# ross39/new_bloom_filter_repo

Measured on AMD Instinct MI355X. Metric: Mpixels/s Bloom insert+query, 1080p residuals, higher is better.
Workload: dtype u64

## Files before the change

new_bloom_filter_repo_amd/csrc/rbf_api.hip:

```cpp
#include "rbf_host.h"
#include "rbf_kernels_noise.h"
#include "rbf_kernels_pack.h"
#include "rbf_rice_host.h"

#include <cmath>

struct MaskArgs {
    const void *frames; FrameLayout l; uint32_t nframes;
    int32_t thr_floor; const int32_t *thr_floors;
    void *masks; uint64_t mask_stride; uint64_t *ones;
    uint32_t channels;
};

static int launch_finish_ones(rbf_ctx *ctx, uint64_t *ones_dev, uint32_t pairs, uint64_t *host_block, uint64_t token,
                              void *clear_a, size_t bytes_a, void *clear_b, size_t bytes_b)
{
    if (clear_a && (((uintptr_t)clear_a | bytes_a) & 15)) { HIP_TRY(hipMemsetAsync(clear_a, 0, bytes_a, ctx->stream)); clear_a = nullptr; bytes_a = 0; }
    if (clear_b && (((uintptr_t)clear_b | bytes_b) & 15)) { HIP_TRY(hipMemsetAsync(clear_b, 0, bytes_b, ctx->stream)); clear_b = nullptr; bytes_b = 0; }
    const uint64_t quads = bytes_a / 16 + bytes_b / 16;
    uint32_t blocks = (uint32_t)((quads + 256 * 4 - 1) / (256 * 4));
    if (blocks < 1) blocks = 1;
    if (blocks > 1024) blocks = 1024;
    hipLaunchKernelGGL(k_finish_ones, dim3(blocks), dim3(256), 0, ctx->stream, ctx->ones_acc.p, ones_dev, pairs, host_block, token,
                       (uint4 *)clear_a, (uint64_t)(bytes_a / 16), (uint4 *)clear_b, (uint64_t)(bytes_b / 16));
// ... 575 lines not shown
    LaunchTimer t(ctx, scatter ? RBF_K_SCATTER : RBF_K_GATHER);
    if (int r = count_and_scan_masks(ctx, mask_dev, 0, n, 1, count_dev)) return r;
    by_sample_width(sample_bytes, [&](auto s) {
        using S = decltype(s);
        auto kern = scatter ? k_values<S, true> : k_values<S, false>;
        hipLaunchKernelGGL(kern, grid, block, 0, ctx->stream, (uint8_t *)frame_dev, width, n, row_pitch_bytes, pixel_stride_bytes, channels,
                           (const uint64_t *)mask_dev, ctx->seg_off.p, nseg, (S *)values_dev);
    });
    HIP_TRY(hipGetLastError());
    return RBF_OK;
}

extern "C" {

int rbf_version(void) { return RBF_ABI_VERSION; }
const char *rbf_last_error(void) { return g_err; }

int rbf_device_count(int *count)
{
    if (!count) return fail(RBF_EINVAL, "count is null");
    int c = 0;
    hipError_t e = hipGetDeviceCount(&c);
    if (e != hipSuccess) { *count = 0; return fail(RBF_EIO, "hipGetDeviceCount: %s", hipGetErrorString(e)); }
    *count = c;
    return RBF_OK;
}

int rbf_ctx_create(int device, void *hip_stream, rbf_ctx **out)
{
    if (!out) return fail(RBF_EINVAL, "out is null");
    *out = nullptr;
    int count = 0;
    HIP_TRY(hipGetDeviceCount(&count));
    if (device < 0 || device >= count) return fail(RBF_EINVAL, "device %d out of range (have %d)", device, count);
    HIP_TRY(hipSetDevice(device));
    rbf_ctx *c = new (std::nothrow) rbf_ctx();
    if (!c) return fail(RBF_ENOMEM, "out of host memory");
    c->device = device;
    int cus = 0;
    if (hipDeviceGetAttribute(&cus, hipDeviceAttributeMultiprocessorCount, device) == hipSuccess && cus > 0) c->cus = (uint32_t)cus;
    if (hip_stream) { c->stream = (hipStream_t)hip_stream; c->owns_stream = false; }
    else {
        hipError_t e = hipStreamCreateWithFlags(&c->stream, hipStreamNonBlocking);
        if (e != hipSuccess) { delete c; return fail(RBF_EIO, "hipStreamCreate: %s", hipGetErrorString(e)); }
        c->owns_stream = true;
    }
    *out = c;
    return RBF_OK;
}

int rbf_ctx_destroy(rbf_ctx *ctx)
{
    if (!ctx) return RBF_OK;
    (void)hipSetDevice(ctx->device);
    (void)hipStreamSynchronize(ctx->stream);
    for (auto &t : ctx->pending) { (void)hipEventDestroy(t.a); (void)hipEventDestroy(t.b); }
    for (auto e : ctx->pool) (void)hipEventDestroy(e);
    hash_table_release(ctx);
    if (ctx->owns_stream) (void)hipStreamDestroy(ctx->stream);
    delete ctx;
    return RBF_OK;
}

int rbf_ctx_sync(rbf_ctx *ctx)
{
    if (int r = set_device(ctx)) return r;
    HIP_TRY(hipStreamSynchronize(ctx->stream));
    return RBF_OK;
}

int rbf_malloc(rbf_ctx *ctx, size_t bytes, void **out_dev)
{
    if (int r = set_device(ctx)) return r;
    if (!out_dev) return fail(RBF_EINVAL, "out_dev is null");
    *out_dev = nullptr;
    if (bytes == 0) bytes = 8;
    hipError_t e = hipMalloc(out_dev, bytes);
    if (e != hipSuccess) return fail(e == hipErrorOutOfMemory ? RBF_ENOMEM : RBF_EIO, "hipMalloc(%zu): %s", bytes, hipGetErrorString(e));
    return RBF_OK;
}

int rbf_free(rbf_ctx *ctx, void *ptr_dev)
{
    if (int r = set_device(ctx)) return r;
    if (!ptr_dev) return RBF_OK;
    HIP_TRY(hipStreamSynchronize(ctx->stream));
    HIP_TRY(hipFree(ptr_dev));
    return RBF_OK;
}

int rbf_memset(rbf_ctx *ctx, void *dst_dev, int value, size_t bytes)
{
    if (int r = set_device(ctx)) return r;
    if (bytes == 0) return RBF_OK;
    if (!dst_dev) return fail(RBF_EINVAL, "dst_dev is null");
    HIP_TRY(hipMemsetAsync(dst_dev, value, bytes, ctx->stream));
    return RBF_OK;
}

int rbf_memcpy_h2d(rbf_ctx *ctx, void *dst_dev, const void *src, size_t bytes)
{
    if (int r = set_device(ctx)) return r;
    if (bytes == 0) return RBF_OK;
    if (!dst_dev || !src) return fail(RBF_EINVAL, "null pointer");
    HIP_TRY(hipMemcpyAsync(dst_dev, src, bytes, hipMemcpyHostToDevice, ctx->stream));
    HIP_TRY(hipStreamSynchronize(ctx->stream));
    return RBF_OK;
}

int rbf_memcpy_d2h(rbf_ctx *ctx, void *dst, const void *src_dev, size_t bytes)
{
    if (int r = set_device(ctx)) return r;
    if (bytes == 0) return RBF_OK;
    if (!dst || !src_dev) return fail(RBF_EINVAL, "null pointer");
    HIP_TRY(hipMemcpyAsync(dst, src_dev, bytes, hipMemcpyDeviceToHost, ctx->stream));
    HIP_TRY(hipStreamSynchronize(ctx->stream));
    return RBF_OK;
}

int rbf_memcpy_d2d(rbf_ctx *ctx, void *dst_dev, const void *src_dev, size_t bytes)
{
    if (int r = set_device(ctx)) return r;
    if (bytes == 0) return RBF_OK;
    if (!dst_dev || !src_dev) return fail(RBF_EINVAL, "null pointer");
    HIP_TRY(hipMemcpyAsync(dst_dev, src_dev, bytes, hipMemcpyDeviceToDevice, ctx->stream));
    return RBF_OK;
}

int rbf_timing_enable(rbf_ctx *ctx, int on)
{
    if (int r = set_device(ctx)) return r;
    if (!on) { if (int r = drain_timing(ctx)) return r; }
    ctx->timing = on == 1 ? 0xFFFFFFFFu : (uint32_t)on;
    return RBF_OK;
}

int rbf_ctx_force_generic(rbf_ctx *ctx, int on)
{
    if (!ctx) return fail(RBF_EINVAL, "null context");
    ctx->knobs.set_flags(on);
    return RBF_OK;
}

int rbf_ctx_option(rbf_ctx *ctx, int option, int64_t value)
{
    if (!ctx) return fail(RBF_EINVAL, "null context");
    switch (option) {
    case RBF_OPT_SEPARATE_FINISH: ctx->knobs.no_fused_finish = value != 0; return RBF_OK;
    case RBF_OPT_INSERT_SLICES: ctx->knobs.insert_slices = value < 0 ? 0u : (uint32_t)value; return RBF_OK;
    default: return fail(RBF_EINVAL, "unknown option %d", option);
    }
}

int rbf_timing_reset(rbf_ctx *ctx)
{
    if (int r = set_device(ctx)) return r;
    if (int r = drain_timing(ctx)) return r;
    for (int k = 0; k < RBF_K_COUNT; ++k) { ctx->total_ms[k] = 0; ctx->launches[k] = 0; }
    return RBF_OK;
}

int rbf_timing_read(rbf_ctx *ctx, int kernel_id, double *total_ms, uint64_t *launches)
{
    if (int r = set_device(ctx)) return r;
    if (kernel_id < 0 || kernel_id >= RBF_K_COUNT) return fail(RBF_EINVAL, "kernel id %d", kernel_id);
    if (int r = drain_timing(ctx)) return r;
    if (total_ms) *total_ms = ctx->total_ms[kernel_id];
    if (launches) *launches = ctx->launches[kernel_id];
    return RBF_OK;
}

int rbf_optimal_params(uint64_t n, uint64_t ones, double *k_out, uint64_t *l_out)
{
    if (!k_out || !l_out) return fail(RBF_EINVAL, "null output");
    *k_out = 0.0; *l_out = 0;
    if (n == 0 || ones > n) return fail(RBF_EINVAL, "need 0 <= ones <= n, n > 0");
    const double p = (double)ones / (double)n;
    if (p <= 0.0001) return RBF_OK;
    if (p >= 0.32453) return RBF_OK;
    const double q = 1 - p;
    const double L = std::log(2.0);
    const double k = std::log2(q * std::pow(L, 2.0) / p);
    if (std::isnan(k) || k <= 0) return RBF_OK;
    const double gamma = 1 / L;
    const double lf = p * (double)n * k * gamma;
    const uint64_t l = (uint64_t)lf;
    *k_out = k > 0.1 ? k : 0.1;
    *l_out = l > 1 ? l : 1;
    return RBF_OK;
}

int rbf_activation_threshold(double k_star, uint32_t *floor_k, uint64_t *threshold)
{
    if (!floor_k || !threshold) return fail(RBF_EINVAL, "null output");
    if (!(k_star >= 0.0) || k_star > 64.0) return fail(RBF_ERANGE, "k* = %g outside [0, 64]", k_star);
    const double fl = std::floor(k_star);
    *floor_k = (uint32_t)fl;
    const double pa = k_star - fl;
    if (!(pa > 0.0)) { *threshold = 0; return RBF_OK; }
    int ex;
    const double fr = std::frexp(pa, &ex);
    const uint64_t A = (uint64_t)std::ldexp(fr, 53);
    const int s = ex - 53 - 2;
    const uint64_t N = (A == (1ull << 52)) ? 4 * A - 1 : 4 * A - 2;
    const int sh = -s;
    if (sh >= 128) { *threshold = 1; return RBF_OK; }
    const unsigned __int128 X = (unsigned __int128)N * (unsigned __int128)0xFFFFFFFFFFFFFFFFull;
    *threshold = (uint64_t)(X >> sh) + 1;
    return RBF_OK;
}

int rbf_plan_batch(uint64_t n, const uint64_t *ones, uint32_t nframes, int guard_l_ge_n,
                   rbf_filter_params *params, double *k_out)
{
    if (!ones || !params) return fail(RBF_EINVAL, "null pointer");
    for (uint32_t f = 0; f < nframes; ++f) {
        double k = 0.0; uint64_t l = 0;
        if (int r = rbf_optimal_params(n, ones[f], &k, &l)) return r;
        const bool skip = (l == 0) || (guard_l_ge_n && l >= n) || l > 0xFFFFFFFFull;
        params[f].m = 0; params[f].floor_k = 0; params[f].threshold = 0;
        if (!skip) {
            params[f].m = (uint32_t)l;
            if (int r = rbf_activation_threshold(k, &params[f].floor_k, &params[f].threshold)) return r;
        }
        if (k_out) k_out[f] = skip ? 0.0 : k;
    }
    return RBF_OK;
}

int rbf_residual_mask_batch(rbf_ctx *ctx, const void *frames_dev, uint64_t frame_stride_bytes,
                            uint32_t nframes, uint32_t width, uint32_t height,
                            uint64_t row_pitch_bytes, uint32_t pixel_stride_bytes,
                            uint32_t sample_bytes, int32_t thr_floor, const int32_t *thr_floors,
                            void *masks_dev, uint64_t mask_stride_bytes, uint64_t *ones_dev)
{
    return rbf_residual_mask_batch_ex(ctx, frames_dev, frame_stride_bytes, nframes, width, height, row_pitch_bytes, pixel_stride_bytes, sample_bytes,
                                      thr_floor, thr_floors, masks_dev, mask_stride_bytes, ones_dev, 1);
}

int rbf_residual_mask_batch_ex(rbf_ctx *ctx, const void *frames_dev, uint64_t frame_stride_bytes,
                               uint32_t nframes, uint32_t width, uint32_t height,
                               uint64_t row_pitch_bytes, uint32_t pixel_stride_bytes,
                               uint32_t sample_bytes, int32_t thr_floor, const int32_t *thr_floors,
                               void *masks_dev, uint64_t mask_stride_bytes, uint64_t *ones_dev, uint32_t mask_channels)
{
    const FrameLayout l{width, height, row_pitch_bytes, pixel_stride_bytes, sample_bytes, frame_stride_bytes};
    return residual_mask_impl(ctx, MaskArgs{frames_dev, l, nframes, thr_floor, thr_floors, masks_dev, mask_stride_bytes, ones_dev, mask_channels}, true);
}

int rbf_bgr_to_gray_batch(rbf_ctx *ctx, const void *frames_dev, uint64_t frame_stride_bytes, uint32_t nframes,
                          uint32_t width, uint32_t height, uint64_t row_pitch_bytes, uint32_t pixel_stride_bytes,
                          uint32_t sample_bytes, void *gray_dev)
{
    const FrameLayout l{width, height, row_pitch_bytes, pixel_stride_bytes, sample_bytes, frame_stride_bytes};
    return pixel_pass(ctx, frames_dev, l, nframes, 3, gray_dev, RBF_K_MASK, [](auto s) { return k_bgr_to_gray<decltype(s)>; });
}

int rbf_extract_luma_batch(rbf_ctx *ctx, const void *frames_dev, uint64_t frame_stride_bytes, uint32_t nframes,
                           uint32_t width, uint32_t height, uint64_t row_pitch_bytes, uint32_t pixel_stride_bytes,
                           uint32_t sample_bytes, void *luma_dev)
{
    const FrameLayout l{width, height, row_pitch_bytes, pixel_stride_bytes, sample_bytes, frame_stride_bytes};
    return pixel_pass(ctx, frames_dev, l, nframes, 1, luma_dev, -1, [](auto s) { return k_extract_luma<decltype(s)>; });
}

int rbf_noise_moments_batch(rbf_ctx *ctx, const void *frames_dev, uint64_t frame_stride_bytes,
                            uint32_t nframes, uint32_t width, uint32_t height,
                            uint64_t row_pitch_bytes, uint32_t pixel_stride_bytes,
                            uint32_t sample_bytes, int64_t *moments_dev, float *noise_dev)
{
    if (int r = set_device(ctx)) return r;
    if (!frames_dev || !moments_dev) return fail(RBF_EINVAL, "null device pointer");
    const FrameLayout l{width, height, row_pitch_bytes, pixel_stride_bytes, sample_bytes, frame_stride_bytes};
    if (int r = check_layout(l, nframes, frame_pass_rules(1))) return r;
    if ((uint64_t)width * height >= (1ull << 32)) return fail(RBF_ERANGE, "frame of %llu pixels is too large", (unsigned long long)width * height);
    const uint32_t by = (height + NZ_TILE_H - 1) / NZ_TILE_H;
    if (by > 65535) return fail(RBF_ERANGE, "frame height %u too large", height);
    HIP_TRY(hipMemsetAsync(moments_dev, 0, (size_t)nframes * 2 * sizeof(int64_t), ctx->stream));
    const dim3 grid((width + NZ_TILE_W - 1) / NZ_TILE_W, by, nframes), block(NZ_THREADS);
    LaunchTimer t(ctx, RBF_K_NOISE);
    by_sample_width(sample_bytes, [&](auto s) {
        hipLaunchKernelGGL(k_noise_moments<decltype(s)>, grid, block, 0, ctx->stream, (const uint8_t *)frames_dev, frame_stride_bytes, width, height,
                           row_pitch_bytes, pixel_stride_bytes, (unsigned long long *)moments_dev, noise_dev);
    });
    HIP_TRY(hipGetLastError());
    return RBF_OK;
}

int rbf_bloom_encode_batch(rbf_ctx *ctx, const void *masks_dev, uint64_t mask_stride_bytes,
                           uint64_t n, uint32_t nframes, const rbf_filter_params *params,
                           const rbf_seeds *seeds,
                           void *filters_dev, uint64_t filter_stride_bytes,
                           void *witnesses_dev, uint64_t witness_stride_bytes,
                           uint64_t *stats_dev)
{
    return encode_batch_impl(ctx, BloomBatch{(void *)masks_dev, mask_stride_bytes, n, nframes, params, seeds, filters_dev, filter_stride_bytes,
                                             witnesses_dev, witness_stride_bytes, stats_dev}, false);
}

int rbf_encode_gop(rbf_ctx *ctx, const void *frames_dev, uint64_t frame_stride_bytes,
                   uint32_t nframes, uint32_t width, uint32_t height,
                   uint64_t row_pitch_bytes, uint32_t pixel_stride_bytes,
                   uint32_t sample_bytes, int32_t thr_floor, const int32_t *thr_floors,
                   const rbf_seeds *seeds,
                   void *masks_dev, uint64_t mask_stride_bytes, uint64_t *ones_dev,
                   void *filters_dev, uint64_t filter_stride_bytes,
// ... 461 lines not shown
```

new_bloom_filter_repo_amd/csrc/rbf_kernels_i64.h:

```cpp
#pragma once
#include "rbf_kernels_q64.h"

namespace rbf {

constexpr int HT_THREADS = 256;

__global__ __launch_bounds__(HT_THREADS) void k_hash_table(uint64_t n, Seeds seeds, uint4 *__restrict__ table)
{
    const uint32_t lane = threadIdx.x & 63u, wave = threadIdx.x >> 6;
    const uint64_t seg = (uint64_t)blockIdx.x * (HT_THREADS / WAVE) + wave;
    if (seg * QL_SEG_PIXELS >= n) return;
    const uint64_t i0 = seg * QL_SEG_PIXELS + (uint64_t)lane * QL_P;
    uint64_t h1[QL_P], h2[QL_P], ha[QL_P];
    uint32_t validmask = 0;
#pragma unroll
    for (int it = 0; it < QL_P; ++it) {
        h1[it] = 0; h2[it] = 0; ha[it] = 0;
        if (i0 + it < n) validmask |= 1u << it;
    }
    if (!hash3_run8((uint32_t)i0, validmask, seeds, h1, h2, ha)) {
#pragma unroll
        for (int it = 0; it < QL_P; ++it) {
            const bool act = (validmask >> it) & 1u;
            const Hash3 h = hash3_index((uint32_t)(i0 + it), act, seeds);
            h1[it] = h.h1; h2[it] = h.h2; ha[it] = h.ha;
        }
    }
    hash_table_store8(table, n, seg, lane, h1, h2, ha);
}

constexpr int IT_STEP_BYTES = 128;
constexpr int IT_CHUNK_STEPS = 16;
constexpr int IT_QUEUE = 64 + IT_STEP_BYTES * 8;
constexpr int IT_STAGE_BYTES = IT_CHUNK_STEPS * IT_STEP_BYTES;
constexpr int IT_WAVE_LDS_BYTES = IT_QUEUE * 2 + IT_STAGE_BYTES;
static_assert(IT_WAVE_LDS_BYTES % 16 == 0 && (IT_QUEUE * 2) % 16 == 0, "the stage is written by LDS-DMA");

template <bool RECORDS, int NWAVES, bool HASHED = false, bool WHOLE = false>
__device__ __forceinline__ void insert_tab_steps(const uint8_t *__restrict__ mask , uint64_t row_bytes , uint64_t n,
                                                 const FrameDev &fd, const uint4 *__restrict__ table, const Seeds &seeds,
                                                 uint32_t *filt, uint32_t tile_bit0, uint32_t tile_bits, uint2 *__restrict__ records, uint32_t rpos,
                                                 uint32_t *wave_lds , uint64_t g0, uint64_t g1, uint32_t lane, uint32_t wave)
{
    static_assert((NWAVES & (NWAVES - 1)) == 0, "a power of two");
    uint16_t *q = reinterpret_cast<uint16_t *>(wave_lds);
    const uint32_t stage = __builtin_amdgcn_readfirstlane(lds_addr_of(wave_lds) + IT_QUEUE * 2);
    uint32_t qn = 0;
    const uint32_t m = vgpr_copy(__builtin_amdgcn_readfirstlane(fd.m));
    const uint32_t fk = __builtin_amdgcn_readfirstlane(fd.floor_k);
    const double ninv = __builtin_bit_cast(double, fd.M);
    const uint64_t T = fd.T;
    auto set_bit = [&](uint32_t pos) {
        if (WHOLE) { atomicOr(&filt[pos >> 5], msb_bit(pos)); return; }
        const uint32_t rel = pos - tile_bit0;
        if (rel < tile_bits) atomicOr(&filt[rel >> 5], msb_bit(pos));
    };

    const HashTable tv(const_cast<uint4 *>(table), n);
    const uint32_t Ttag = (uint32_t)(T >> 48);
    uint4 e0 = make_uint4(0, 0, 0, 0);
    uint32_t tag = 0, slot_kept = 0;
    uint64_t ha_kept = 0;
    uint32_t pending = 0;
    uint32_t cb = 0;
    auto fetch = [&](uint32_t first, uint32_t count) {
        const uint32_t e = lane < count ? q[first + lane] : 0u;
        const uint32_t idx = ((cb + (e >> 10) * NWAVES) << 10) + (e & 1023u);
        if (HASHED) {
            const Hash3 h = hash3_index(idx, lane < count, seeds);
            e0 = make_uint4((uint32_t)h.h1, (uint32_t)(h.h1 >> 32), (uint32_t)h.h2, (uint32_t)(h.h2 >> 32));
            tag = (uint32_t)(h.ha >> 48);
            ha_kept = h.ha;
        } else {
            slot_kept = hash_table_slot(idx);
            e0 = tv.pos[slot_kept];
            tag = tv.tag[idx];
        }
        pending = count;
    };
    auto finish = [&]() {
        if (!pending) return;
        if (lane < pending) {
            uint32_t pos = mod_m_f64(rn_double(e0.x, e0.y), e0.x, ninv, m);
            const uint32_t step = mod_m_f64(rn_double(e0.z, e0.w), e0.z, ninv, m);
            bool act = tag < Ttag;
            if (tag == Ttag) act = (HASHED ? ha_kept : tv.act[slot_kept]) < T;
            if (RECORDS) {
                records[rpos + lane] = make_uint2(pos, step | (act ? 0x80000000u : 0u));
            } else {
                for (uint32_t j = 0; j < fk; ++j) {
                    set_bit(pos);
                    const uint32_t s2 = pos + step;
                    pos = min(s2, s2 - m);
                }
                if (act) set_bit(pos);
            }
        }
        if (RECORDS) rpos += pending;
        pending = 0;
    };

    const uint32_t nbytes32 = (uint32_t)((n + 7) >> 3), n32 = (uint32_t)n, row32 = (uint32_t)row_bytes;
    const uint32_t gend = (uint32_t)g1;
    auto staged = [&](uint32_t s) -> uint32_t {
        return *reinterpret_cast<const __attribute__((address_space(3))) uint16_t *>((uintptr_t)(stage + s * IT_STEP_BYTES + lane * 2u));
    };
    auto decode = [&](uint32_t v, uint32_t g) -> uint32_t {
        const uint32_t byte = g * IT_STEP_BYTES + lane * 2u;
        const uint32_t x = __builtin_bitreverse32(v) >> 16;
        uint32_t b = ((x & 0xFFu) << 8) | (x >> 8);
        const uint32_t rem = n32 - byte * 8u;
        if (rem < 16u) b &= (1u << rem) - 1u;
        return (g < gend && byte < nbytes32) ? b : 0u;
    };
    for (uint32_t chunk = __builtin_amdgcn_readfirstlane((uint32_t)g0 + wave); chunk < gend; chunk += NWAVES * IT_CHUNK_STEPS) {
        cb = chunk;
        wave_lds_fence();
#pragma unroll
        for (int i = 0; i < IT_CHUNK_STEPS / 2; ++i) {
            const uint32_t g = cb + (2u * i + (lane >> 5)) * NWAVES;
            const uint32_t off = g * IT_STEP_BYTES + (lane & 31u) * 4u;
            if (g < gend && off < row32) {
                const uint32_t dst = stage + (uint32_t)i * 256u;
                uint32_t keep;
                asm volatile("s_mov_b32 %0, m0\n\ts_mov_b32 m0, %1\n\ts_nop 0\n\tglobal_load_lds_dword %2, %3\n\ts_mov_b32 m0, %0"
                             : "=&s"(keep) : "s"(dst), "v"(off), "s"(mask) : "memory");
            }
        }
        dma_wait_all();
        wave_lds_fence();
        uint32_t nxt = staged(0);
        for (uint32_t s = 0; s < IT_CHUNK_STEPS && cb + s * NWAVES < gend; ++s) {
            const uint32_t g = cb + s * NWAVES;
            uint32_t bits = decode(nxt, g);
            nxt = staged(s + 1 < IT_CHUNK_STEPS ? s + 1 : s);
            const uint32_t c = __popc(bits);
            const uint32_t incl = wave_inclusive_scan(c);
            const uint32_t excl = incl - c;
            const uint32_t total = __builtin_amdgcn_readlane(incl, 63);
            uint32_t off = qn + excl;
            const uint32_t ebase = (s << 10) | (lane << 4);
            while (bits) {
                q[off++] = (uint16_t)(ebase + __builtin_ctz(bits));
                bits &= bits - 1u;
            }
            qn += total;
            wave_lds_fence();
            while (qn >= WAVE) {
                qn -= WAVE;
                finish();
                fetch(qn, WAVE);
            }
            wave_lds_fence();
        }
        if (cb + NWAVES * IT_CHUNK_STEPS < gend && qn) {
            finish();
            fetch(0, qn);
            qn = 0;
            wave_lds_fence();
        }
    }
    finish();
    if (qn) { fetch(0, qn); finish(); }
}

template <bool HASHED = false, bool WHOLE = false>
__global__ __launch_bounds__(IL_THREADS) void k_insert_tab(
    const uint8_t *__restrict__ masks, uint64_t mask_stride_bytes, uint64_t n,
    const FrameTable tab, const uint4 *__restrict__ table , Seeds seeds,
    uint32_t *__restrict__ partials, uint64_t part_stride_words32, uint32_t tile_words ,
    const SliceTable slices, uint32_t per_tile , uint32_t Smax )
{
    extern __shared__ __attribute__((aligned(16))) uint32_t lds[];
    uint32_t *filt = lds;
    uint32_t *queues = lds + tile_words;
    const uint32_t tile = blockIdx.x / per_tile;
    uint32_t s = blockIdx.x - tile * per_tile, f = 0;
    while (s >= slices.n[f]) { s -= slices.n[f]; ++f; }
    const uint32_t S = slices.n[f];
    const FrameDev fd = tab.f[f];
    if (fd.m == 0) return;
    const uint32_t lane = threadIdx.x & 63u, wave = threadIdx.x >> 6;
    const uint32_t fwords = filter_words(fd.m);
    const uint32_t tile0 = tile * tile_words;
    if (tile0 >= fwords) return;
    for (uint32_t i = threadIdx.x; i < tile_words; i += IL_THREADS) filt[i] = 0;
    __syncthreads();

    const uint64_t nbytes = (n + 7) >> 3;
    const uint64_t groups = (nbytes + IT_STEP_BYTES - 1) / IT_STEP_BYTES;
    const uint64_t gper = (groups + S - 1) / S;
    const uint64_t g0 = (uint64_t)s * gper;
    const uint64_t g1 = g0 + gper < groups ? g0 + gper : groups;
    insert_tab_steps<false, IL_WAVES, HASHED, WHOLE>(masks + (uint64_t)f * mask_stride_bytes, mask_stride_bytes, n, fd, table, seeds, filt, tile0 << 5, tile_words << 5, nullptr, 0u,
                                                     queues + wave * (IT_WAVE_LDS_BYTES / 4), g0, g1, lane, wave);
    __syncthreads();
    uint32_t *part = partials + ((uint64_t)f * Smax + s) * part_stride_words32 + tile0;
    const uint32_t mine = fwords - tile0 < tile_words ? fwords - tile0 : tile_words;
    const uint32_t pairs = (mine + 1) >> 1;
    for (uint32_t i = threadIdx.x; i < pairs; i += IL_THREADS)
        reinterpret_cast<uint2 *>(part)[i] = reinterpret_cast<const uint2 *>(filt)[i];
}

constexpr int IP_THREADS = 256, IP_WAVES = IP_THREADS / WAVE;

template <bool HASHED = false>
__global__ __launch_bounds__(IP_THREADS) void k_insert_positions(
    const uint8_t *__restrict__ masks, uint64_t mask_stride_bytes, uint64_t n,
    const FrameTable tab , const uint4 *__restrict__ table , Seeds seeds,
    uint2 *__restrict__ records, uint32_t *__restrict__ counters )
{
    __shared__ __attribute__((aligned(16))) uint32_t queues[IP_WAVES * (IT_WAVE_LDS_BYTES / 4)];
    const uint32_t f = blockIdx.y, s = blockIdx.x, S = gridDim.x;
    const FrameDev fd = tab.f[f];
    if (fd.m == 0) return;
    const uint32_t lane = threadIdx.x & 63u, wave = threadIdx.x >> 6;
    const uint64_t nbytes = (n + 7) >> 3;
    const uint64_t groups = (nbytes + IT_STEP_BYTES - 1) / IT_STEP_BYTES;
    const uint64_t gper = (groups + S - 1) / S;
    const uint64_t g0 = (uint64_t)s * gper;
    const uint64_t g1 = g0 + gper < groups ? g0 + gper : groups;
    const uint8_t *mask = masks + (uint64_t)f * mask_stride_bytes;
    __shared__ uint32_t wcount[IP_WAVES];
    __shared__ uint32_t wg_base;
    uint32_t mine = 0;
    for (uint64_t g = g0 + wave; g < g1; g += IP_WAVES) {
        const uint64_t byte = g * IT_STEP_BYTES + lane * 2;
        if (byte < nbytes) {
            uint32_t v = *reinterpret_cast<const uint16_t *>(mask + byte);
            const uint64_t rem = n - byte * 8;
            if (rem < 16) {
                const uint32_t x = __builtin_bitreverse32(v) >> 16;
                v = (((x & 0xFFu) << 8) | (x >> 8)) & ((1u << rem) - 1u);
            }
            mine += __popc(v);
        }
    }
    const uint32_t wave_total = __builtin_amdgcn_readlane(wave_inclusive_scan(mine), 63);
    if (lane == 0) wcount[wave] = wave_total;
    __syncthreads();
    if (threadIdx.x == 0) {
        uint32_t t = 0;
        for (int k = 0; k < IP_WAVES; ++k) t += wcount[k];
        wg_base = t ? atomicAdd(counters + f, t) : 0u;
    }
    __syncthreads();
    uint32_t rpos = wg_base;
    for (uint32_t k = 0; k < wave; ++k) rpos += wcount[k];
    insert_tab_steps<true, IP_WAVES, HASHED>(mask, mask_stride_bytes, n, fd, table, seeds, nullptr, 0u, 0u, records + fd.floor_k, (uint32_t)__builtin_amdgcn_readfirstlane((int)rpos),
                                             queues + wave * (IT_WAVE_LDS_BYTES / 4), g0, g1, lane, wave);
}

constexpr int IR_UNROLL = 4;

__global__ __launch_bounds__(IL_THREADS) void k_insert_records(
    const uint2 *__restrict__ records, const uint32_t *__restrict__ counters, const FrameTable tab ,
    uint32_t *__restrict__ partials, uint64_t part_stride_words32, uint32_t tile_words ,
    const SliceTable slices, uint32_t per_tile , uint32_t Smax)
{
    extern __shared__ __attribute__((aligned(16))) uint32_t lds[];
    const uint32_t tile = blockIdx.x / per_tile;
    uint32_t s = blockIdx.x - tile * per_tile, f = 0;
    while (s >= slices.n[f]) { s -= slices.n[f]; ++f; }
    const uint32_t S = slices.n[f];
    const uint32_t m = tab.f[f].m;
    if (m == 0) return;
    const uint32_t fk = tab.f[f].floor_k;
    const uint32_t fwords = filter_words(m);
    const uint32_t tile0 = tile * tile_words;
    if (tile0 >= fwords) return;
    const uint32_t tile_bit0 = tile0 << 5, tile_bits = tile_words << 5;
    for (uint32_t i = threadIdx.x; i < tile_words; i += IL_THREADS) lds[i] = 0;
    __syncthreads();
    const uint32_t count = counters[f];
    const uint32_t per = (((count + S - 1) / S) + 63u) & ~63u;
    const uint32_t r0 = s * per < count ? s * per : count, r1 = r0 + per < count ? r0 + per : count;
    const uint2 *rec = records + tab.f[f].T;
    auto insert = [&](uint2 r) {
        uint32_t pos = r.x;
        const uint32_t step = r.y & 0x7FFFFFFFu;
        for (uint32_t j = 0; j < fk; ++j) {
            const uint32_t rel = pos - tile_bit0;
            if (rel < tile_bits) atomicOr(&lds[rel >> 5], msb_bit(pos));
            const uint32_t s2 = pos + step;
            pos = min(s2, s2 - m);
        }
        const uint32_t rel = pos - tile_bit0;
        if ((r.y >> 31) && rel < tile_bits) atomicOr(&lds[rel >> 5], msb_bit(pos));
    };
    uint32_t i = r0 + threadIdx.x;
    for (; i + (IR_UNROLL - 1) * IL_THREADS < r1; i += IR_UNROLL * IL_THREADS) {
        uint2 r[IR_UNROLL];
#pragma unroll
        for (int u = 0; u < IR_UNROLL; ++u) r[u] = rec[i + u * IL_THREADS];
#pragma unroll
        for (int u = 0; u < IR_UNROLL; ++u) insert(r[u]);
    }
    for (; i < r1; i += IL_THREADS) insert(rec[i]);
    __syncthreads();
    uint32_t *part = partials + ((uint64_t)f * Smax + s) * part_stride_words32 + tile0;
    const uint32_t mine = fwords - tile0 < tile_words ? fwords - tile0 : tile_words;
    const uint32_t pairs = (mine + 1) >> 1;
    for (uint32_t k = threadIdx.x; k < pairs; k += IL_THREADS)
        reinterpret_cast<uint2 *>(part)[k] = reinterpret_cast<const uint2 *>(lds)[k];
}

}
```

new_bloom_filter_repo_amd/csrc/rbf_kernels_lds.h:

```cpp
#pragma once
#include "rbf_kernels.h"

namespace rbf {

typedef uint32_t nt_u32x4 __attribute__((ext_vector_type(4)));
__device__ __forceinline__ void store_stream(uint4 *p, uint4 v) { const nt_u32x4 x = {v.x, v.y, v.z, v.w}; __builtin_nontemporal_store(x, reinterpret_cast<nt_u32x4 *>(p)); }
__device__ __forceinline__ uint4 load_stream(const uint4 *p) { const nt_u32x4 x = __builtin_nontemporal_load(reinterpret_cast<const nt_u32x4 *>(p)); return make_uint4(x.x, x.y, x.z, x.w); }

constexpr int QL_THREADS = 1024;
constexpr int QL_WAVES = QL_THREADS / WAVE;
constexpr int QL_P = 8;
constexpr int QL_SEG_PIXELS = QL_P * WAVE;

constexpr int IL_THREADS = 1024;
constexpr int IL_WAVES = IL_THREADS / WAVE;
constexpr int IL_QUEUE = 64 + 512;

__device__ __forceinline__ void wave_lds_fence()
{
    __builtin_amdgcn_fence(__ATOMIC_RELEASE, "wavefront");
    __builtin_amdgcn_wave_barrier();
    __builtin_amdgcn_fence(__ATOMIC_ACQUIRE, "wavefront");
}

__device__ __forceinline__ uint32_t mod_m_small(uint64_t h, uint32_t m, uint32_t m2, uint32_t Mh, uint32_t Ml)
{
    const uint32_t hh = (uint32_t)(h >> 32), hl = (uint32_t)h;
    const uint32_t q = hh * Mh + __umulhi(hh, Ml) + __umulhi(hl, Mh);
    uint32_t r = hl - q * m;
    r = min(r, r - m2);
    r = min(r, r - m);
    return r;
}

template <bool SMALL_M>
__global__ __launch_bounds__(IL_THREADS) void k_insert_lds(
    const uint8_t *__restrict__ masks, uint64_t mask_stride_bytes, uint64_t n,
    const FrameTable tab, Seeds seeds,
    uint32_t *__restrict__ partials, uint64_t part_stride_words32, uint32_t tile_words ,
    const SliceTable slices, uint32_t per_tile , uint32_t Smax )
{
    extern __shared__ __attribute__((aligned(16))) uint32_t lds[];
    uint32_t *filt = lds;
    uint32_t *queues = lds + tile_words;
    const uint32_t tile = blockIdx.x / per_tile;
    uint32_t s = blockIdx.x - tile * per_tile, f = 0;
    while (s >= slices.n[f]) { s -= slices.n[f]; ++f; }
    const uint32_t S = slices.n[f];
    const FrameDev fd = tab.f[f];
    if (fd.m == 0) return;
    const uint32_t lane = threadIdx.x & 63u, wave = threadIdx.x >> 6;
    const uint32_t fwords = filter_words(fd.m);
    const uint32_t tile0 = tile * tile_words;
    if (tile0 >= fwords) return;
    const uint32_t tile_bit0 = tile0 << 5, tile_bits = tile_words << 5;
    for (uint32_t i = threadIdx.x; i < tile_words; i += IL_THREADS) filt[i] = 0;
    __syncthreads();

    const uint8_t *mask = masks + (uint64_t)f * mask_stride_bytes;
    const uint64_t nbytes = (n + 7) >> 3;
    const uint64_t groups = (nbytes + 63) >> 6;
    const uint64_t gper = (groups + S - 1) / S;
    const uint64_t g0 = (uint64_t)s * gper;
    const uint64_t g1 = g0 + gper < groups ? g0 + gper : groups;
    uint32_t *q = queues + wave * IL_QUEUE;
    uint32_t qn = 0;

    const uint32_t m = fd.m, m2 = fd.m << 1, Mh = (uint32_t)(fd.M >> 32), Ml = (uint32_t)fd.M;
    auto drain_at = [&](uint32_t first, uint32_t count) {
        const bool act = lane < count;
        const uint32_t idx = act ? q[first + lane] : 0u;
        const Hash3 h = hash3_index(idx, act, seeds);
        if (act) {
            uint32_t pos, step;
            if (SMALL_M) { pos = mod_m_small(h.h1, m, m2, Mh, Ml); step = mod_m_small(h.h2, m, m2, Mh, Ml); }
            else         { pos = mod_m(h.h1, m, fd.M);             step = mod_m(h.h2, m, fd.M); }
            for (uint32_t j = 0; j < fd.floor_k; ++j) {
                const uint32_t rel = pos - tile_bit0;
                if (rel < tile_bits) atomicOr(&filt[rel >> 5], msb_bit(pos));
                const uint64_t s2 = (uint64_t)pos + step;
                pos = (uint32_t)(s2 >= m ? s2 - m : s2);
            }
            const uint32_t rel = pos - tile_bit0;
            if (h.ha < fd.T && rel < tile_bits) atomicOr(&filt[rel >> 5], msb_bit(pos));
        }
    };

    auto load_bits = [&](uint64_t g) -> uint32_t {
        const uint64_t byte = g * 64 + lane;
        if (g >= g1 || byte >= nbytes) return 0u;
        uint32_t b = __builtin_bitreverse32((uint32_t)mask[byte]) >> 24;
        const uint64_t rem = n - byte * 8;
        if (rem < 8) b &= (1u << rem) - 1u;
        return b;
    };
    uint32_t nxt = load_bits(g0 + wave);
    for (uint64_t g = g0 + wave; g < g1; g += IL_WAVES) {
        uint32_t bits = nxt;
        nxt = load_bits(g + IL_WAVES);
        const uint32_t c = __popc(bits);
        const uint64_t b0 = __ballot((c & 1u) != 0), b1 = __ballot((c & 2u) != 0);
        const uint64_t b2 = __ballot((c & 4u) != 0), b3 = __ballot((c & 8u) != 0);
        const uint32_t excl = rank_below(b0) + 2u * rank_below(b1) + 4u * rank_below(b2) + 8u * rank_below(b3);
        const uint32_t total = __popcll(b0) + 2u * __popcll(b1) + 4u * __popcll(b2) + 8u * __popcll(b3);
        uint32_t off = qn + excl;
        const uint32_t base = (uint32_t)((g * 64 + lane) << 3);
        while (bits) {
            q[off++] = base + __builtin_ctz(bits);
            bits &= bits - 1u;
        }
        qn += total;
        wave_lds_fence();
        while (qn >= WAVE) {
            qn -= WAVE;
            drain_at(qn, WAVE);
        }
        wave_lds_fence();
    }
    drain_at(0, qn);
    __syncthreads();
    uint32_t *part = partials + ((uint64_t)f * Smax + s) * part_stride_words32 + tile0;
    const uint32_t mine = fwords - tile0 < tile_words ? fwords - tile0 : tile_words;
    const uint32_t pairs = (mine + 1) >> 1;
    for (uint32_t i = threadIdx.x; i < pairs; i += IL_THREADS)
        reinterpret_cast<uint2 *>(part)[i] = reinterpret_cast<const uint2 *>(filt)[i];
}

template <bool STREAM>
__global__ __launch_bounds__(WG_THREADS) void k_filter_reduce(
    const uint32_t *partials, uint64_t part_stride_words32, uint32_t Smax ,
    const SliceTable slices ,
    const FrameTable tab,
    uint32_t *filters , uint64_t filter_stride_words32,
    uint64_t *__restrict__ stats, uint32_t vec_ok,
    uint32_t *__restrict__ image , uint64_t image_stride_words32)
{
    __shared__ uint32_t red[WG_WAVES];
    const uint32_t f = blockIdx.y;
    const uint32_t S = slices.n[f];
    const uint32_t m = tab.f[f].m;
    const uint32_t fwords = m ? filter_words(m) : 0u;
    uint32_t *filt = filters + (uint64_t)f * filter_stride_words32;
    const uint32_t *part = partials + (uint64_t)f * Smax * part_stride_words32;
    uint32_t pc = 0;
    if (vec_ok) {
        const uint64_t quads = filter_stride_words32 >> 2;
        for (uint64_t q = (uint64_t)blockIdx.x * WG_THREADS + threadIdx.x; q < quads; q += (uint64_t)gridDim.x * WG_THREADS) {
            const uint64_t w = q << 2;
            uint4 v = make_uint4(0, 0, 0, 0);
            if (w < fwords) {
                for (uint32_t s0 = 0; s0 < S; s0 += 8) {
                    uint4 x[8];
#pragma unroll
                    for (int j = 0; j < 8; ++j) {
                        const uint32_t sj = s0 + j < S ? s0 + j : S - 1;
                        const uint4 *src = reinterpret_cast<const uint4 *>(part + (uint64_t)sj * part_stride_words32 + w);
                        x[j] = STREAM ? load_stream(src) : *src;
                    }
#pragma unroll
                    for (int j = 0; j < 8; ++j) { v.x |= x[j].x; v.y |= x[j].y; v.z |= x[j].z; v.w |= x[j].w; }
                }
                if (w + 1 >= fwords) v.y = 0;
                if (w + 2 >= fwords) v.z = 0;
                if (w + 3 >= fwords) v.w = 0;
            }
            if (m) {
                if (STREAM) store_stream(reinterpret_cast<uint4 *>(filt + w), v); else *reinterpret_cast<uint4 *>(filt + w) = v;
            }
            if (image && w < image_stride_words32)
                *reinterpret_cast<uint4 *>(image + (uint64_t)f * image_stride_words32 + w) =
                    make_uint4(~__builtin_bswap32(v.x), ~__builtin_bswap32(v.y), ~__builtin_bswap32(v.z), ~__builtin_bswap32(v.w));
            pc += __popc(v.x) + __popc(v.y) + __popc(v.z) + __popc(v.w);
        }
    } else {
        for (uint64_t w = (uint64_t)blockIdx.x * WG_THREADS + threadIdx.x; w < filter_stride_words32; w += (uint64_t)gridDim.x * WG_THREADS) {
            uint32_t v = 0;
            if (w < fwords)
                for (uint32_t s = 0; s < S; ++s) v |= part[(uint64_t)s * part_stride_words32 + w];
            if (m) filt[w] = v;
            if (image && w < image_stride_words32) image[(uint64_t)f * image_stride_words32 + w] = ~__builtin_bswap32(v);
            pc += __popc(v);
        }
    }
#pragma unroll
    for (int d = 32; d >= 1; d >>= 1) pc += __shfl_down(pc, d);
    if ((threadIdx.x & 63u) == 0) red[threadIdx.x >> 6] = pc;
    __syncthreads();
    if (threadIdx.x == 0) {
        uint32_t t = 0;
        for (int k = 0; k < WG_WAVES; ++k) t += red[k];
        if (t) atomicAdd((unsigned long long *)&stats[(uint64_t)f * 4 + 1], (unsigned long long)t);
    }
}

__global__ __launch_bounds__(WG_THREADS) void k_probe_image(const uint32_t *__restrict__ filters, uint64_t filter_stride_words32,
                                                            uint32_t *__restrict__ image, uint64_t image_stride_words32)
{
    const uint32_t f = blockIdx.y;
    for (uint64_t w = (uint64_t)blockIdx.x * WG_THREADS + threadIdx.x; w < image_stride_words32; w += (uint64_t)gridDim.x * WG_THREADS)
        image[(uint64_t)f * image_stride_words32 + w] = w < filter_stride_words32 ? ~__builtin_bswap32(filters[(uint64_t)f * filter_stride_words32 + w]) : ~0u;
}

__device__ __forceinline__ void dma16(const uint32_t *gsrc, uint32_t lds_byte_addr)
{
    uint32_t keep;
    asm volatile("s_mov_b32 %0, m0\n\t"
                 "s_mov_b32 m0, %2\n\t"
                 "s_nop 0\n\t"
                 "global_load_lds_dwordx4 %1, off\n\t"
                 "s_mov_b32 m0, %0"
                 : "=&s"(keep) : "v"(gsrc), "s"(lds_byte_addr) : "memory");
}
__device__ __forceinline__ void dma4(const uint32_t *gsrc, uint32_t lds_byte_addr)
{
    uint32_t keep;
    asm volatile("s_mov_b32 %0, m0\n\t"
                 "s_mov_b32 m0, %2\n\t"
                 "s_nop 0\n\t"
                 "global_load_lds_dword %1, off\n\t"
                 "s_mov_b32 m0, %0"
                 : "=&s"(keep) : "v"(gsrc), "s"(lds_byte_addr) : "memory");
}
__device__ __forceinline__ void dma_wait_all() { asm volatile("s_waitcnt vmcnt(0)" ::: "memory"); }

__device__ __forceinline__ uint32_t lds_addr_of(const uint32_t *p)
{
    return (uint32_t)(uintptr_t)(const __attribute__((address_space(3))) uint32_t *)p;
}

__device__ __forceinline__ void dma_filter(uint32_t *lds_dst, const uint32_t *src, uint32_t words, uint32_t wave,
                                           uint32_t lane, uint32_t nwaves)
{
    const uint32_t base = __builtin_amdgcn_readfirstlane(lds_addr_of(lds_dst));
    const uint32_t npieces = words >> 2;
    const uint32_t nchunks = (npieces + 63u) >> 6;
    for (uint32_t c = wave; c < nchunks; c += nwaves) {
        const uint32_t piece = (c << 6) + lane;
        if (piece < npieces) dma16(src + (piece << 2), __builtin_amdgcn_readfirstlane(base + (c << 10)));
    }
    const uint32_t tail = words & 3u;
    if (wave == 0 && lane < tail) dma4(src + (npieces << 2) + lane, __builtin_amdgcn_readfirstlane(base + (npieces << 4)));
}

__device__ __forceinline__ void valu_sgpr_hazard_gap(uint32_t (&a)[8], uint32_t (&b)[8])
{
    asm volatile("" : "+s"(a[0]), "+s"(a[1]), "+s"(a[2]), "+s"(a[3]), "+s"(a[4]), "+s"(a[5]), "+s"(a[6]), "+s"(a[7]));
    asm volatile("s_nop 4" : "+s"(b[0]), "+s"(b[1]), "+s"(b[2]), "+s"(b[3]), "+s"(b[4]), "+s"(b[5]), "+s"(b[6]), "+s"(b[7]));
}
__device__ __forceinline__ void write_lane(uint32_t &dst, uint32_t uniform_value, int lane_index)
{
    asm volatile("v_writelane_b32 %0, %1, %2" : "+v"(dst) : "s"(uniform_value), "n"(lane_index));
}

__device__ __forceinline__ uint32_t probe_word(const uint32_t *filt, uint32_t pos)
{
    const uint32_t w = __builtin_amdgcn_ubfe(pos, 5, 27);
    return filt[w];
}

template <bool SMALL_M, int FK>
__device__ __forceinline__ uint32_t frame_pass(
    const uint64_t (&h1)[QL_P], const uint64_t (&h2)[QL_P], const uint64_t (&ha)[QL_P], uint32_t validmask,
    const uint32_t *filt, uint32_t m, uint64_t M, uint64_t T, uint32_t fk_rt, uint32_t &pb)
{
    const uint32_t Mh = (uint32_t)(M >> 32), Ml = (uint32_t)M;
    const uint32_t fk = FK >= 0 ? (uint32_t)FK : fk_rt;
    const uint32_t m2 = m << 1;
    uint32_t npass = 0;
    pb = 0;
#pragma unroll
    for (int it = 0; it < QL_P; ++it) {
        uint32_t pos, step;
        if (SMALL_M) { pos = mod_m_small(h1[it], m, m2, Mh, Ml); step = mod_m_small(h2[it], m, m2, Mh, Ml); }
        else         { pos = mod_m(h1[it], m, M);            step = mod_m(h2[it], m, M); }
        uint32_t acc = validmask << (31 - it);
#pragma unroll
        for (uint32_t j = 0; j < fk; ++j) {
            acc &= probe_word(filt, pos) << ((pos ^ 24u) & 31u);
// ... 590 lines not shown
```

Baseline: 557,600.

## Prestage first mask chunk before LDS clear and vectorize slice lookup and stores

The insert kernel now issues the LDS-DMA load of its first mask chunk before zeroing the filter tile, so the global load overlaps the clear and the barrier. The tile clear and the partial-filter store widen to 16-byte accesses. The serial frame/slice search loop is replaced by a wave-wide scan and ballot. The tail flush is reordered so the last fetch is issued before the in-flight batch finishes. Optional timestamp probes are added behind a compile flag. The wider stores assume tile sizes are multiples of four words, and the scan assumes the batch fits in two frames per lane.

```diff
diff --git a/new_bloom_filter_repo_amd/csrc/rbf_api.hip b/new_bloom_filter_repo_amd/csrc/rbf_api.hip
--- a/new_bloom_filter_repo_amd/csrc/rbf_api.hip
+++ b/new_bloom_filter_repo_amd/csrc/rbf_api.hip
@@ -751,6 +751,17 @@
     }
 }
 
+#ifdef RBF_INSERT_PHASE_STAMPS
+int rbf_debug_insert_stamps(rbf_ctx *ctx, void *host, size_t bytes)
+{
+    if (int r = set_device(ctx)) return r;
+    HIP_TRY(hipStreamSynchronize(ctx->stream));
+    if (bytes > sizeof(uint64_t) * IT_STAMP_WGS * 16 * IT_STAMPS) return fail(RBF_EINVAL, "stamp buffer is smaller");
+    HIP_TRY(hipMemcpyFromSymbol(host, HIP_SYMBOL(rbf::g_it_stamps), bytes, 0, hipMemcpyDeviceToHost));
+    return RBF_OK;
+}
+#endif
+
 int rbf_timing_reset(rbf_ctx *ctx)
 {
     if (int r = set_device(ctx)) return r;
diff --git a/new_bloom_filter_repo_amd/csrc/rbf_kernels_i64.h b/new_bloom_filter_repo_amd/csrc/rbf_kernels_i64.h
--- a/new_bloom_filter_repo_amd/csrc/rbf_kernels_i64.h
+++ b/new_bloom_filter_repo_amd/csrc/rbf_kernels_i64.h
@@ -36,7 +36,37 @@
 constexpr int IT_WAVE_LDS_BYTES = IT_QUEUE * 2 + IT_STAGE_BYTES;
 static_assert(IT_WAVE_LDS_BYTES % 16 == 0 && (IT_QUEUE * 2) % 16 == 0, "the stage is written by LDS-DMA");
 
-template <bool RECORDS, int NWAVES, bool HASHED = false, bool WHOLE = false>
+#ifdef RBF_INSERT_PHASE_STAMPS
+constexpr int IT_STAMPS = 9, IT_STAMP_WGS = 1024;
+__device__ uint64_t g_it_stamps[IT_STAMP_WGS * 16 * IT_STAMPS];
+__device__ __forceinline__ void it_stamp(int k)
+{
+    if ((threadIdx.x & 63u) == 0 && blockIdx.x < (uint32_t)IT_STAMP_WGS)
+        g_it_stamps[((uint64_t)blockIdx.x * 16 + (threadIdx.x >> 6)) * IT_STAMPS + k] = wall_clock64();
+}
+#define RBF_IT_STAMP(k) it_stamp(k)
+#else
+#define RBF_IT_STAMP(k) ((void)0)
+#endif
+
+template <int NWAVES>
+__device__ __forceinline__ void it_stage_chunk(const uint8_t *__restrict__ mask , uint32_t stage ,
+                                               uint32_t cb, uint32_t gend, uint32_t row32, uint32_t lane)
+{
+#pragma unroll
+    for (int i = 0; i < IT_CHUNK_STEPS / 2; ++i) {
+        const uint32_t g = cb + (2u * i + (lane >> 5)) * NWAVES;
+        const uint32_t off = g * IT_STEP_BYTES + (lane & 31u) * 4u;
+        if (g < gend && off < row32) {
+            const uint32_t dst = stage + (uint32_t)i * 256u;
+            uint32_t keep;
+            asm volatile("s_mov_b32 %0, m0\n\ts_mov_b32 m0, %1\n\ts_nop 0\n\tglobal_load_lds_dword %2, %3\n\ts_mov_b32 m0, %0"
+                         : "=&s"(keep) : "s"(dst), "v"(off), "s"(mask) : "memory");
+        }
+    }
+}
+
+template <bool RECORDS, int NWAVES, bool HASHED = false, bool WHOLE = false, bool PRESTAGED = false>
 __device__ __forceinline__ void insert_tab_steps(const uint8_t *__restrict__ mask , uint64_t row_bytes , uint64_t n,
                                                  const FrameDev &fd, const uint4 *__restrict__ table, const Seeds &seeds,
                                                  uint32_t *filt, uint32_t tile_bit0, uint32_t tile_bits, uint2 *__restrict__ records, uint32_t rpos,
@@ -58,33 +88,36 @@
 
     const HashTable tv(const_cast<uint4 *>(table), n);
     const uint32_t Ttag = (uint32_t)(T >> 48);
-    uint4 e0 = make_uint4(0, 0, 0, 0);
-    uint32_t tag = 0, slot_kept = 0;
-    uint64_t ha_kept = 0;
-    uint32_t pending = 0;
+    struct Batch {
+        uint4 e0 = make_uint4(0, 0, 0, 0);
+        uint32_t tag = 0, slot_kept = 0;
+        uint64_t ha_kept = 0;
+        uint32_t pending = 0;
+    };
+    Batch flight;
     uint32_t cb = 0;
-    auto fetch = [&](uint32_t first, uint32_t count) {
+    auto fetch = [&](Batch &bt, uint32_t first, uint32_t count) {
         const uint32_t e = lane < count ? q[first + lane] : 0u;
         const uint32_t idx = ((cb + (e >> 10) * NWAVES) << 10) + (e & 1023u);
         if (HASHED) {
             const Hash3 h = hash3_index(idx, lane < count, seeds);
-            e0 = make_uint4((uint32_t)h.h1, (uint32_t)(h.h1 >> 32), (uint32_t)h.h2, (uint32_t)(h.h2 >> 32));
-            tag = (uint32_t)(h.ha >> 48);
-            ha_kept = h.ha;
+            bt.e0 = make_uint4((uint32_t)h.h1, (uint32_t)(h.h1 >> 32), (uint32_t)h.h2, (uint32_t)(h.h2 >> 32));
+            bt.tag = (uint32_t)(h.ha >> 48);
+            bt.ha_kept = h.ha;
         } else {
-            slot_kept = hash_table_slot(idx);
-            e0 = tv.pos[slot_kept];
-            tag = tv.tag[idx];
-        }
-        pending = count;
-    };
-    auto finish = [&]() {
-        if (!pending) return;
-        if (lane < pending) {
-            uint32_t pos = mod_m_f64(rn_double(e0.x, e0.y), e0.x, ninv, m);
-            const uint32_t step = mod_m_f64(rn_double(e0.z, e0.w), e0.z, ninv, m);
-            bool act = tag < Ttag;
-            if (tag == Ttag) act = (HASHED ? ha_kept : tv.act[slot_kept]) < T;
+            bt.slot_kept = hash_table_slot(idx);
+            bt.e0 = tv.pos[bt.slot_kept];
+            bt.tag = tv.tag[idx];
+        }
+        bt.pending = count;
+    };
+    auto finish = [&](Batch &bt) {
+        if (!bt.pending) return;
+        if (lane < bt.pending) {
+            uint32_t pos = mod_m_f64(rn_double(bt.e0.x, bt.e0.y), bt.e0.x, ninv, m);
+            const uint32_t step = mod_m_f64(rn_double(bt.e0.z, bt.e0.w), bt.e0.z, ninv, m);
+            bool act = bt.tag < Ttag;
+            if (bt.tag == Ttag) act = (HASHED ? bt.ha_kept : tv.act[bt.slot_kept]) < T;
             if (RECORDS) {
                 records[rpos + lane] = make_uint2(pos, step | (act ? 0x80000000u : 0u));
             } else {
@@ -96,8 +129,8 @@
                 if (act) set_bit(pos);
             }
         }
-        if (RECORDS) rpos += pending;
-        pending = 0;
+        if (RECORDS) rpos += bt.pending;
+        bt.pending = 0;
     };
 
     const uint32_t nbytes32 = (uint32_t)((n + 7) >> 3), n32 = (uint32_t)n, row32 = (uint32_t)row_bytes;
@@ -113,22 +146,17 @@
         if (rem < 16u) b &= (1u << rem) - 1u;
         return (g < gend && byte < nbytes32) ? b : 0u;
     };
+    bool staged_by_caller = PRESTAGED;
     for (uint32_t chunk = __builtin_amdgcn_readfirstlane((uint32_t)g0 + wave); chunk < gend; chunk += NWAVES * IT_CHUNK_STEPS) {
         cb = chunk;
-        wave_lds_fence();
-#pragma unroll
-        for (int i = 0; i < IT_CHUNK_STEPS / 2; ++i) {
-            const uint32_t g = cb + (2u * i + (lane >> 5)) * NWAVES;
-            const uint32_t off = g * IT_STEP_BYTES + (lane & 31u) * 4u;
-            if (g < gend && off < row32) {
-                const uint32_t dst = stage + (uint32_t)i * 256u;
-                uint32_t keep;
-                asm volatile("s_mov_b32 %0, m0\n\ts_mov_b32 m0, %1\n\ts_nop 0\n\tglobal_load_lds_dword %2, %3\n\ts_mov_b32 m0, %0"
-                             : "=&s"(keep) : "s"(dst), "v"(off), "s"(mask) : "memory");
-            }
-        }
+        if (!staged_by_caller) {
+            wave_lds_fence();
+            it_stage_chunk<NWAVES>(mask, stage, cb, gend, row32, lane);
+        }
+        staged_by_caller = false;
         dma_wait_all();
         wave_lds_fence();
+        RBF_IT_STAMP(3);
         uint32_t nxt = staged(0);
         for (uint32_t s = 0; s < IT_CHUNK_STEPS && cb + s * NWAVES < gend; ++s) {
             const uint32_t g = cb + s * NWAVES;
@@ -148,20 +176,24 @@
             wave_lds_fence();
             while (qn >= WAVE) {
                 qn -= WAVE;
-                finish();
-                fetch(qn, WAVE);
+                finish(flight);
+                fetch(flight, qn, WAVE);
             }
             wave_lds_fence();
         }
         if (cb + NWAVES * IT_CHUNK_STEPS < gend && qn) {
-            finish();
-            fetch(0, qn);
+            finish(flight);
+            fetch(flight, 0, qn);
             qn = 0;
             wave_lds_fence();
         }
     }
-    finish();
-    if (qn) { fetch(0, qn); finish(); }
+    RBF_IT_STAMP(4);
+    Batch last;
+    if (qn) fetch(last, 0, qn);
+    finish(flight);
+    finish(last);
+    RBF_IT_STAMP(5);
 }
 
 template <bool HASHED = false, bool WHOLE = false>
@@ -174,9 +206,10 @@
     extern __shared__ __attribute__((aligned(16))) uint32_t lds[];
     uint32_t *filt = lds;
     uint32_t *queues = lds + tile_words;
+    RBF_IT_STAMP(0);
     const uint32_t tile = blockIdx.x / per_tile;
-    uint32_t s = blockIdx.x - tile * per_tile, f = 0;
-    while (s >= slices.n[f]) { s -= slices.n[f]; ++f; }
+    uint32_t s, f;
+    slice_coords(slices, blockIdx.x - tile * per_tile, f, s);
     const uint32_t S = slices.n[f];
     const FrameDev fd = tab.f[f];
     if (fd.m == 0) return;
@@ -184,22 +217,33 @@
     const uint32_t fwords = filter_words(fd.m);
     const uint32_t tile0 = tile * tile_words;
     if (tile0 >= fwords) return;
-    for (uint32_t i = threadIdx.x; i < tile_words; i += IL_THREADS) filt[i] = 0;
-    __syncthreads();
-
+    RBF_IT_STAMP(1);
     const uint64_t nbytes = (n + 7) >> 3;
     const uint64_t groups = (nbytes + IT_STEP_BYTES - 1) / IT_STEP_BYTES;
     const uint64_t gper = (groups + S - 1) / S;
     const uint64_t g0 = (uint64_t)s * gper;
     const uint64_t g1 = g0 + gper < groups ? g0 + gper : groups;
-    insert_tab_steps<false, IL_WAVES, HASHED, WHOLE>(masks + (uint64_t)f * mask_stride_bytes, mask_stride_bytes, n, fd, table, seeds, filt, tile0 << 5, tile_words << 5, nullptr, 0u,
-                                                     queues + wave * (IT_WAVE_LDS_BYTES / 4), g0, g1, lane, wave);
-    __syncthreads();
+    const uint8_t *mask = masks + (uint64_t)f * mask_stride_bytes;
+    uint32_t *wave_lds = queues + wave * (IT_WAVE_LDS_BYTES / 4);
+    if ((uint32_t)g0 + wave < (uint32_t)g1)
+        it_stage_chunk<IL_WAVES>(mask, __builtin_amdgcn_readfirstlane(lds_addr_of(wave_lds) + IT_QUEUE * 2), __builtin_amdgcn_readfirstlane((uint32_t)g0 + wave),
+                                 (uint32_t)g1, (uint32_t)mask_stride_bytes, lane);
+    for (uint32_t i = threadIdx.x; i < tile_words >> 2; i += IL_THREADS) reinterpret_cast<uint4 *>(filt)[i] = make_uint4(0, 0, 0, 0);
+    __syncthreads();
+    RBF_IT_STAMP(2);
+
+    insert_tab_steps<false, IL_WAVES, HASHED, WHOLE, true>(mask, mask_stride_bytes, n, fd, table, seeds, filt, tile0 << 5, tile_words << 5, nullptr, 0u,
+                                                                wave_lds, g0, g1, lane, wave);
+    __syncthreads();
+    RBF_IT_STAMP(6);
     uint32_t *part = partials + ((uint64_t)f * Smax + s) * part_stride_words32 + tile0;
     const uint32_t mine = fwords - tile0 < tile_words ? fwords - tile0 : tile_words;
-    const uint32_t pairs = (mine + 1) >> 1;
-    for (uint32_t i = threadIdx.x; i < pairs; i += IL_THREADS)
-        reinterpret_cast<uint2 *>(part)[i] = reinterpret_cast<const uint2 *>(filt)[i];
+    tile_store16(part, filt, mine);
+    RBF_IT_STAMP(7);
+#ifdef RBF_INSERT_PHASE_STAMPS
+    dma_wait_all();
+    RBF_IT_STAMP(8);
+#endif
 }
 
 constexpr int IP_THREADS = 256, IP_WAVES = IP_THREADS / WAVE;
@@ -260,8 +304,8 @@
 {
     extern __shared__ __attribute__((aligned(16))) uint32_t lds[];
     const uint32_t tile = blockIdx.x / per_tile;
-    uint32_t s = blockIdx.x - tile * per_tile, f = 0;
-    while (s >= slices.n[f]) { s -= slices.n[f]; ++f; }
+    uint32_t s, f;
+    slice_coords(slices, blockIdx.x - tile * per_tile, f, s);
     const uint32_t S = slices.n[f];
     const uint32_t m = tab.f[f].m;
     if (m == 0) return;
@@ -300,9 +344,7 @@
     __syncthreads();
     uint32_t *part = partials + ((uint64_t)f * Smax + s) * part_stride_words32 + tile0;
     const uint32_t mine = fwords - tile0 < tile_words ? fwords - tile0 : tile_words;
-    const uint32_t pairs = (mine + 1) >> 1;
-    for (uint32_t k = threadIdx.x; k < pairs; k += IL_THREADS)
-        reinterpret_cast<uint2 *>(part)[k] = reinterpret_cast<const uint2 *>(lds)[k];
-}
-
-}
+    tile_store16(part, lds, mine);
+}
+
+}
diff --git a/new_bloom_filter_repo_amd/csrc/rbf_kernels_lds.h b/new_bloom_filter_repo_amd/csrc/rbf_kernels_lds.h
--- a/new_bloom_filter_repo_amd/csrc/rbf_kernels_lds.h
+++ b/new_bloom_filter_repo_amd/csrc/rbf_kernels_lds.h
@@ -33,6 +33,25 @@
     return r;
 }
 
+__device__ __forceinline__ void slice_coords(const SliceTable &slices, uint32_t idx, uint32_t &f, uint32_t &s)
+{
+    static_assert(MAX_BATCH == 2 * WAVE, "two frames per lane");
+    const uint32_t lane = threadIdx.x & 63u;
+    const uint32_t a = slices.n[2u * lane], b = slices.n[2u * lane + 1u];
+    const uint32_t incl = wave_inclusive_scan(a + b), mid = incl - b;
+    const uint32_t nf = (uint32_t)__popcll(__ballot(mid <= idx)) + (uint32_t)__popcll(__ballot(incl <= idx));
+    const uint32_t before = (nf & 1u) ? mid : incl - a - b;
+    f = nf;
+    s = idx - (uint32_t)__builtin_amdgcn_readlane((int)before, (int)(nf >> 1));
+}
+
+__device__ __forceinline__ void tile_store16(uint32_t *__restrict__ part, const uint32_t *filt , uint32_t mine)
+{
+    const uint32_t quads = (mine + 3) >> 2;
+    for (uint32_t i = threadIdx.x; i < quads; i += blockDim.x)
+        reinterpret_cast<uint4 *>(part)[i] = reinterpret_cast<const uint4 *>(filt)[i];
+}
+
 template <bool SMALL_M>
 __global__ __launch_bounds__(IL_THREADS) void k_insert_lds(
     const uint8_t *__restrict__ masks, uint64_t mask_stride_bytes, uint64_t n,
@@ -44,8 +63,8 @@
     uint32_t *filt = lds;
     uint32_t *queues = lds + tile_words;
     const uint32_t tile = blockIdx.x / per_tile;
-    uint32_t s = blockIdx.x - tile * per_tile, f = 0;
-    while (s >= slices.n[f]) { s -= slices.n[f]; ++f; }
+    uint32_t s, f;
+    slice_coords(slices, blockIdx.x - tile * per_tile, f, s);
     const uint32_t S = slices.n[f];
     const FrameDev fd = tab.f[f];
     if (fd.m == 0) return;
@@ -121,9 +140,7 @@
     __syncthreads();
     uint32_t *part = partials + ((uint64_t)f * Smax + s) * part_stride_words32 + tile0;
     const uint32_t mine = fwords - tile0 < tile_words ? fwords - tile0 : tile_words;
-    const uint32_t pairs = (mine + 1) >> 1;
-    for (uint32_t i = threadIdx.x; i < pairs; i += IL_THREADS)
-        reinterpret_cast<uint2 *>(part)[i] = reinterpret_cast<const uint2 *>(filt)[i];
+    tile_store16(part, filt, mine);
 }
 
 template <bool STREAM>
```

Result: no change. 561,400, median of 6 (+0.7%).
